# NoemieJaquier/GaBOtorch

Measured on AMD Instinct MI355X. Metric: SPD affine-invariant kernel-matrix build, pairs/sec (N=4096,d=10), higher is better.
Workload: dtype f64

## Files before the change

### gabotorch_amd/csrc/spd_pairwise_body.hpp

```cpp
#pragma once
#include "gabo_device.hpp"
#include "spd_eig.hpp"
#include "spd_prep.hpp"
#include "gabo_mirror.hpp"
#include "spd_generic.hpp"
#include "gabo_log_tab.hpp"
#include "gabo_exp_tab256.hpp"
#include "gabo_acosh2_table.hpp"
#include "../../include/gabo_hip.h"

#ifndef GABO_PAIR_WAVES
#define GABO_PAIR_WAVES 2
#endif

namespace gabo {

typedef const double __attribute__((address_space(1)))* spd_gcol_ptr;

struct SpdGcolBuffer {
    __amdgpu_buffer_rsrc_t rsrc;
    int voff;
    int stride_bytes;
    __device__ __forceinline__ double operator[](int k) const {
        return __builtin_bit_cast(double, __builtin_amdgcn_raw_buffer_load_b64(rsrc, voff, k * stride_bytes, 0));
    }
};
struct SpdGcolPointer {
    spd_gcol_ptr p;
    int64_t stride;
    __device__ __forceinline__ double operator[](int k) const { return p[(int64_t)k * stride]; }
};

template <int D, int ORIENT = kQlOrientPerLane, class GCOL>
__device__ __forceinline__ double ai_sumsq(const double* __restrict__ W, const GCOL& Gj, const double* __restrict__ ltab, const double eps2 = 0.0) {
    constexpr int T = tri_size(D);
    constexpr bool kDescending = ORIENT == kQlOrientLast;
    double m[T];
    static_for<D>([&](auto cc) {
        constexpr int col = kDescending ? D - 1 - decltype(cc)::value : decltype(cc)::value;
        double g[D - col], c[D - col];
        static_for<D - col>([&](auto kk) { g[decltype(kk)::value] = Gj[tri(col + decltype(kk)::value, col)]; });
        static_for<D - col>([&](auto rr) {
            constexpr int r = col + decltype(rr)::value;
            double acc = W[tri(r, col)] * g[0];
            static_for<r - col>([&](auto kk) {
                constexpr int k = col + 1 + decltype(kk)::value;
                acc = __builtin_fma(W[tri(r, k)], g[k - col], acc);
            });
            c[r - col] = acc;
        });
        static_for<D - col>([&](auto rr) {
            constexpr int r = col + decltype(rr)::value;
            static_for<r - col + 1>([&](auto qq) {
                constexpr int q = col + decltype(qq)::value;
                m[tri(r, q)] = (kDescending ? col == q : col == 0) ? c[r - col] * c[q - col] : __builtin_fma(c[r - col], c[q - col], m[tri(r, q)]);
            });
        });
    });
    double dg[D], e2[D];
    tridiagonalize<D, ORIENT>(m, dg, e2);
    tridiag_eigenvalues<D, ORIENT>(dg, e2, eps2);
    double s = 0.0;
    const LogTabRegs lr = LogTabRegs::load();
    static_for<D>([&](auto kk) { double lg = log_tab(dg[decltype(kk)::value], lr, ltab); s = __builtin_fma(lg, lg, s); });
    return s;
}

struct Spd2Col {
    double g00, g10, g11, lg;
};
__device__ __forceinline__ double ai_sumsq2(const double* __restrict__ W, const Spd2Col& g, double lw, const LogTabRegs& lr,
                                            const double* __restrict__ ltab, double tiny) {
    const double c00 = W[0] * g.g00, c11 = W[2] * g.g11;
    const double c10 = __builtin_fma(W[1], g.g00, W[2] * g.g10);
    const double m00 = c00 * c00, m10d = (c10 + c10) * c00, m11 = __builtin_fma(c10, c10, c11 * c11);
    const double tr = m00 + m11, df = m00 - m11;
    const double root = sqrt_nz(__builtin_fma(df, df, __builtin_fma(m10d, m10d, tiny)));
    const double l1 = log_tab(0.5 * (tr + root), lr, ltab);
    const double l2 = __builtin_fma(2.0, lw + g.lg, -l1);
    return __builtin_fma(l1, l1, l2 * l2);
}

__device__ __forceinline__ double finish(double dist, double beta, int mode) {
    if (mode == GABO_OUT_DISTANCE) return dist;
    if (mode == GABO_OUT_LAPLACE) return exp(-(dist * beta));
    return exp(-((dist * dist) * beta));
}

#ifndef GABO_PAIR_TWO_WAVE_MAX_DIM
#define GABO_PAIR_TWO_WAVE_MAX_DIM 14
#endif
#ifndef GABO_QL_EPS2_GAUSS
#define GABO_QL_EPS2_GAUSS 1e-14
#endif
constexpr bool spd_pair_gauss_only_instantiated(int d) { return d > 2 && d != 12; }
#ifndef GABO_PAIR_ORIENT
constexpr int spd_pair_gauss_only_orientation(int d) { return d == 14 ? kQlOrientCol0 : kQlOrientLast; }
#else
constexpr int spd_pair_gauss_only_orientation(int d) { return GABO_PAIR_ORIENT; }
#endif
template <int D, bool GAUSS_ONLY, bool BUFFER_ONLY>
__global__ __launch_bounds__(256, (D > GABO_PAIR_TWO_WAVE_MAX_DIM ? 1 : GABO_PAIR_WAVES)) void spd_ai_pairwise_kernel(const double* __restrict__ Winv, const double* __restrict__ G,
                                                              double* __restrict__ out, double* __restrict__ dist_out_arg,
                                                              int64_t n1, int64_t n2,
                                                              int64_t w_batch_stride, int64_t g_batch_stride, int rows,
                                                              int col_blocks, int row_chunks, int64_t sym_tiles, double beta, int flags) {
    constexpr int T = tri_size(D);
    static_assert(GAUSS_ONLY == BUFFER_ONLY && (spd_pair_gauss_only_instantiated(D) || !GAUSS_ONLY), "instantiations that launch_spd_ai selects");
    const int mode = GAUSS_ONLY ? GABO_OUT_GAUSSIAN : (flags & GABO_OUT_MASK);
    double* const dist_out = GAUSS_ONLY ? nullptr : dist_out_arg;
    constexpr bool kTabExp = D <= 4;
    __shared__ double tab[kTabExp ? 64 : 1];
    __shared__ __attribute__((aligned(16))) double ltab[512];
    for (int k = threadIdx.x; k < 512; k += blockDim.x) ltab[k] = kLogTab[k];
    double ec[6], ec3 = 0.0;
    if constexpr (kTabExp) {
        if (threadIdx.x < 64) tab[threadIdx.x] = kExp2Tab[threadIdx.x];
    }
    __syncthreads();
    if constexpr (kTabExp) {
        static_for<6>([&](auto k) { ec[decltype(k)::value] = kExpTabC[decltype(k)::value]; });
        ec3 = ec[3];
        asm volatile("" : "+v"(ec3));
    }
    int64_t cg, rc, b;
    if (flags & GABO_SYMMETRIC) {
        const int64_t per_batch = sym_tiles;
        b = blockIdx.x / per_batch;
        int64_t t = blockIdx.x - b * per_batch;
        cg = 0;
        for (;;) {
            int64_t cnt = ((cg + 1) * (int64_t)blockDim.x + rows - 1) / rows;
            if (cnt > row_chunks) cnt = row_chunks;
            if (t < cnt) break;
            t -= cnt;
            ++cg;
        }
        rc = t;
    } else {
        const int64_t bid = blockIdx.x;
        cg = bid % col_blocks;
        rc = (bid / col_blocks) % row_chunks;
        b = bid / ((int64_t)col_blocks * row_chunks);
    }
    const int64_t j0 = cg * blockDim.x;
    const int64_t j = j0 + threadIdx.x;
    const int64_t jc = j < n2 ? j : n2 - 1;
    const int64_t i0 = rc * rows;
    const int64_t i1 = (i0 + rows < n1) ? i0 + rows : n1;
    if ((flags & GABO_SYMMETRIC) && j0 + (int64_t)(threadIdx.x | 63) < i0) return;
    const double* Gj = G + b * g_batch_stride + jc;
    double* ob = out + b * n1 * n2;
    const int64_t jw = j0 + (threadIdx.x & ~63);
    const bool use_buffer = BUFFER_ONLY || (D > 2 && (int64_t)T * n2 * 8 < (1ll << 31));
    SpdGcolBuffer gbuf;
    {
        const double* gw = G + b * g_batch_stride + (jw < n2 ? jw : n2 - 1);
        uint64_t a = (uint64_t)gw;
        a = ((uint64_t)(uint32_t)__builtin_amdgcn_readfirstlane((int)(a >> 32)) << 32) | (uint32_t)__builtin_amdgcn_readfirstlane((int)a);
        gbuf.rsrc = __builtin_amdgcn_make_buffer_rsrc((void*)a, 0, 0x7fffffff, 0x00020000);
        gbuf.voff = (int)((jc - (jw < n2 ? jw : n2 - 1)) * 8);
        gbuf.stride_bytes = (int)(n2 * 8);
    }
    Spd2Col col2;
    double lw_lane = 0.0, tiny = 1e-290;
    LogTabRegs lr2;
    if constexpr (D == 2) {
        lr2 = LogTabRegs::load();
        asm volatile("" : "+s"(tiny));
        col2.g00 = Gj[0];
        col2.g10 = Gj[n2];
        col2.g11 = Gj[2 * n2];
        col2.lg = log_tab(col2.g00 * col2.g11, lr2, ltab);
        int64_t ir = i0 + (threadIdx.x & 63);
        ir = ir < n1 ? ir : n1 - 1;
        const double* Wr = Winv + b * w_batch_stride + ir * T;
        lw_lane = log_tab(Wr[0] * Wr[2], lr2, ltab);
    }
    double eps2 = (mode == GABO_OUT_GAUSSIAN && !dist_out) ? GABO_QL_EPS2_GAUSS : 0.0;
    asm volatile("" : "+s"(eps2));
    if constexpr (GAUSS_ONLY && BUFFER_ONLY) {
        const int nrows = __builtin_amdgcn_readfirstlane((int)(i1 - i0));
        const int64_t jrel = j - i0;
        const int rmax = j >= n2 ? -1 : ((flags & GABO_SYMMETRIC) ? (jrel < 0 ? -1 : (jrel > rows - 1 ? rows - 1 : (int)jrel)) : rows - 1);
        const double* W = Winv + b * w_batch_stride + i0 * T;
        char* orow = reinterpret_cast<char*>(ob + i0 * n2 + j);
        for (int r = 0; r < nrows; ++r, W += T) {
            SpdGcolBuffer gb = gbuf;
            asm volatile("" : "+v"(gb.voff));
            asm volatile("" : "+s"(gb.stride_bytes));
            const double s = ai_sumsq<D, spd_pair_gauss_only_orientation(D)>(W, gb, ltab, eps2);
            double val;
            if constexpr (kTabExp) {
                val = exp_neg_tab(-((s + 1e-15) * beta), ec, ec3, tab);
                val = s != s ? s : val;
            } else {
                val = exp(-((s + 1e-15) * beta));
            }
            if (r <= rmax) *reinterpret_cast<double*>(orow) = val;
            orow += (unsigned)gb.stride_bytes;
        }
        return;
    }
    for (int64_t i = i0; i < i1; ++i) {
        const double* W = Winv + b * w_batch_stride + i * T;
        double s;
        if constexpr (D == 2) {
            const int lane = (int)(i - i0);
            const double lw = __hiloint2double(__builtin_amdgcn_readlane(__double2hiint(lw_lane), lane),
                                               __builtin_amdgcn_readlane(__double2loint(lw_lane), lane));
            s = ai_sumsq2(W, col2, lw, lr2, ltab, tiny);
        } else {
            if (use_buffer) {
                SpdGcolBuffer gb = gbuf;
                asm volatile("" : "+v"(gb.voff));
                asm volatile("" : "+s"(gb.stride_bytes));
                s = ai_sumsq<D>(W, gb, ltab, eps2);
            } else {
                SpdGcolPointer gp{(spd_gcol_ptr)Gj, n2};
                asm volatile("" : "+v"(gp.p));
                s = ai_sumsq<D>(W, gp, ltab, eps2);
            }
        }
        double dist, val;
        if (mode == GABO_OUT_GAUSSIAN && !dist_out) {
            dist = 0.0;
            if constexpr (kTabExp) {
                val = exp_neg_tab(-((s + 1e-15) * beta), ec, ec3, tab);
                val = s != s ? s : val;
            } else {
                val = exp(-((s + 1e-15) * beta));
            }
        } else {
            dist = __builtin_sqrt(s + 1e-15);
            val = finish(dist, beta, mode);
        }
        if (j < n2 && (!(flags & GABO_SYMMETRIC) || i <= j)) {
            ob[i * n2 + j] = val;
            if (dist_out) dist_out[b * n1 * n2 + i * n2 + j] = dist;
        }
    }
}

#ifndef GABO_GAUSS2_MAX_ROWS
#define GABO_GAUSS2_MAX_ROWS 64
#endif
constexpr double kGauss2L = 0.0027076061740622863;
__constant__ double kGauss2C[6] = {kGauss2L, kGauss2L * kGauss2L / 2.0, kGauss2L * kGauss2L * kGauss2L / 6.0,
                                   kGauss2L * kGauss2L * kGauss2L * kGauss2L / 24.0, 6755399441055744.0, 4096.0};

template <bool NT, bool SYM>
__global__ __launch_bounds__(256) void spd_ai_gauss2_kernel(const double* __restrict__ Winv, const double* __restrict__ G,
                                                            double* __restrict__ out, int64_t n1, int64_t n2, int64_t w_batch_stride,
                                                            int64_t g_batch_stride, int rows, int col_blocks, int row_chunks,
                                                            int64_t sym_tiles, double beta, int flags) {
    __shared__ __attribute__((aligned(16))) double ltab[512];
    __shared__ double etab[256];
    __shared__ __attribute__((aligned(16))) double atab[kAcosh2Slots * kAcosh2Stride];
    __shared__ __attribute__((aligned(16))) double wrow[GABO_GAUSS2_MAX_ROWS * 4];
    const int tid = threadIdx.x;
    for (int k = tid; k < 512; k += blockDim.x) ltab[k] = kLogTab[k];
    for (int k = tid; k < 256; k += blockDim.x) etab[k] = kExp2Tab256[k];
    {
        const double sc = beta * (-512.0 / 0.69314718055994530942), eps = beta * (-256.0 / 0.69314718055994530942) * 1e-15;
        constexpr int kUsedLo = (kAcosh2Binades - 1) * 16 * kAcosh2Stride, kUsedHi = 240 * kAcosh2Stride;
        for (int k = tid; k < kAcosh2Slots * kAcosh2Stride - (kUsedHi - kUsedLo); k += blockDim.x) {
            const int kk = k < kUsedLo ? k : k + (kUsedHi - kUsedLo);
            const double v = kAcosh2Tab[kk] * sc;
            atab[kk] = (kk % kAcosh2Stride == 0) ? v + eps : v;
        }
    }
    int64_t cg, rc, b;
    if constexpr (SYM) {
        const int64_t per_batch = sym_tiles;
        b = blockIdx.x / per_batch;
        int64_t t = blockIdx.x - b * per_batch;
        cg = 0;
        for (;;) {
            int64_t cnt = ((cg + 1) * (int64_t)blockDim.x + rows - 1) / rows;
            if (cnt > row_chunks) cnt = row_chunks;
            if (t < cnt) break;
            t -= cnt;
            ++cg;
        }
        rc = t;
    } else {
        const int64_t bid = blockIdx.x;
        cg = bid % col_blocks;
        rc = (bid / col_blocks) % row_chunks;
        b = bid / ((int64_t)col_blocks * row_chunks);
    }
    const int64_t j0 = cg * blockDim.x;
    const int64_t j = j0 + tid;
    const int64_t jc = j < n2 ? j : n2 - 1;
    const int64_t i0 = rc * rows;
    const int64_t i1 = (i0 + rows < n1) ? i0 + rows : n1;
    const double* Gj = G + b * g_batch_stride + jc;
    const double g00 = Gj[0], g10 = Gj[n2], g11 = Gj[2 * n2];
    const LogTabRegs lr = LogTabRegs::load();
    const double sscale = __builtin_sqrt(beta * (512.0 / 0.69314718055994530942));
    double w0l = 1.0, w1l = 0.0, w2l = 1.0;
    if (tid < rows) {
        int64_t ir = i0 + tid;
        ir = ir < n1 ? ir : n1 - 1;
        const double* Wr = Winv + b * w_batch_stride + ir * 3;
        w0l = Wr[0], w1l = Wr[1], w2l = Wr[2];
    }
    __syncthreads();
    if (tid < rows) {
        const double dw = w0l * w2l;
        const double sw = rsqrt_nz(dw + dw);
        wrow[4 * tid + 0] = w0l * sw;
        wrow[4 * tid + 1] = w1l * sw;
        wrow[4 * tid + 2] = w2l * sw;
        wrow[4 * tid + 3] = sscale * log_tab(dw, lr, ltab);
    }
    __syncthreads();
    if (SYM && j0 + (int64_t)(tid | 63) < i0) return;
    double ec[6];
    static_for<6>([&](auto k) { ec[decltype(k)::value] = kGauss2C[decltype(k)::value]; });
    double c4v = ec[3];
    asm volatile("" : "+v"(c4v));
    const double dg = g00 * g11;
    const double bcol = sscale * log_tab(dg, lr, ltab);
    const double sg = rsqrt_nz(dg);
    const double q00 = g00 * sg, q10 = g10 * sg, q11 = g11 * sg;
    double* orow = out + b * n1 * n2 + i0 * n2 + j;
    const int nrows = __builtin_amdgcn_readfirstlane((int)(i1 - i0));
    const int64_t jrel = j - i0;
    const int rmax = j >= n2 ? -1 : (SYM ? (jrel < 0 ? -1 : (jrel > GABO_GAUSS2_MAX_ROWS - 1 ? GABO_GAUSS2_MAX_ROWS - 1 : (int)jrel)) : GABO_GAUSS2_MAX_ROWS - 1);
    typedef double g2_v2d __attribute__((ext_vector_type(2)));
    if (!SYM && j >= n2) return;
    for (int r = 0; r < nrows; ++r, orow += n2) {
        const g2_v2d wa = *reinterpret_cast<const g2_v2d*>(wrow + 4 * r);
        const g2_v2d wb = *reinterpret_cast<const g2_v2d*>(wrow + 4 * r + 2);
        const double w0 = wa[0], w1 = wa[1], w2 = wb[0], arow = wb[1];
        const double hh = __builtin_fma(w0, q00, -(w2 * q11));
        const double cc = __builtin_fma(w1, q00, w2 * q10);
        const double tau = __builtin_fma(cc, cc, __builtin_fma(hh, hh, 1.0));
        const unsigned hi = (unsigned)__double2hiint(tau);
        static_assert(kAcosh2MBits == 4 && kAcosh2Slots == 256, "row index = 8 bits");
        const unsigned off = __umul24((hi >> 16) & 0xffu, (unsigned)(kAcosh2Stride * sizeof(double)));
        const double t = tau - __hiloint2double((int)(hi & ~((1u << (20 - kAcosh2MBits)) - 1u)), 0);
        const g2_v2d* row = reinterpret_cast<const g2_v2d*>(reinterpret_cast<const char*>(atab) + off);
        static_assert(kAcosh2Deg == 7, "four coefficient pairs");
        const g2_v2d c67 = row[3], c45 = row[2], c23 = row[1], c01 = row[0];
        double ya = __builtin_fma(c67[1], t, c67[0]);
        ya = __builtin_fma(ya, t, c45[1]);
        ya = __builtin_fma(ya, t, c45[0]);
        ya = __builtin_fma(ya, t, c23[1]);
        ya = __builtin_fma(ya, t, c23[0]);
        ya = __builtin_fma(ya, t, c01[1]);
        ya = __builtin_fma(ya, t, c01[0]);
        if (__builtin_expect(__any(!(tau < ec[5])), 0)) {
            if (!(tau < ec[5])) {
                const double dl = log(tau + __builtin_sqrt(__builtin_fma(tau, tau, -1.0)));
                ya = -(sscale * sscale) * __builtin_fma(dl, dl, 0.5e-15);
            }
        }
        const double sp = arow + bcol;
        const double y = __builtin_fma(-sp, sp, ya);
        const double km = y + ec[4];
        const double kk = km - ec[4];
        const double rr = y - kk;
        double p = __builtin_fma(rr, c4v, ec[2]);
        p = __builtin_fma(p, rr, ec[1]);
        p = __builtin_fma(p, rr, ec[0]);
        p = p * rr;
        const int ki = __double2loint(km);
        const double e = etab[ki & 255];
        const double val = __builtin_ldexp(__builtin_fma(e, p, e), ki >> 8);
        if (!SYM || r <= rmax) {
            if constexpr (NT) __builtin_nontemporal_store(val, orow);
            else *orow = val;
        }
    }
}

template <int D>
static int launch_spd_ai(const double* x1, const double* x2, double* out, double* dist_out, int64_t batch, int64_t n1, int64_t n2,
                         int64_t s1, int64_t s2, double beta, int flags, double* ws, int* status, hipStream_t st, bool prepared = false) {
    constexpr int T = tri_size(D);
    const int64_t b1 = (s1 == 0) ? 1 : batch;
    const int64_t b2 = (s2 == 0) ? 1 : batch;
    double* W = ws;
    double* G = ws + b1 * n1 * T;
    if (!prepared) launch_spd_prep<D>(x1, x2, W, G, b1, b2, n1, n2, s1, s2, status, st, 1);
#ifndef GABO_PAIR_THREADS
#define GABO_PAIR_THREADS (D >= 7 ? 64 : 256)
#endif
    int threads = n2 >= 256 ? GABO_PAIR_THREADS : (n2 > 128 ? 192 : (n2 > 64 ? 128 : 64));
    int64_t col_blocks = (n2 + threads - 1) / threads;
#ifndef GABO_PAIR_ROWS_D2
#define GABO_PAIR_ROWS_D2 16
#endif
#ifndef GABO_PAIR_ROWS
#define GABO_PAIR_ROWS (D >= 9 ? 8 : 16)
#endif
#ifndef GABO_PAIR_ROWS_GAUSS2
#define GABO_PAIR_ROWS_GAUSS2 64
#endif
    const bool gauss2 = D == 2 && (flags & GABO_OUT_MASK) == GABO_OUT_GAUSSIAN && !dist_out && beta >= 0.0;
    int rows = D == 2 ? (gauss2 ? GABO_PAIR_ROWS_GAUSS2 : GABO_PAIR_ROWS_D2) : GABO_PAIR_ROWS;
    while (rows > 1 && col_blocks * ((n1 + rows - 1) / rows) * batch < (rows > 16 ? 1024 : 4096)) rows >>= 1;
    int64_t row_chunks = (n1 + rows - 1) / rows;
    int64_t sym_tiles = 0;
    if (flags & GABO_SYMMETRIC) {
        for (int64_t cg = 0; cg < col_blocks; ++cg) {
            int64_t cnt = ((cg + 1) * threads + rows - 1) / rows;
            sym_tiles += cnt < row_chunks ? cnt : row_chunks;
        }
    }
    int64_t nblocks = ((flags & GABO_SYMMETRIC) ? sym_tiles : col_blocks * row_chunks) * batch;
    if (nblocks > 0x7fffffffLL) return GABO_ERR_ARG;
    bool special2 = false;
    if constexpr (D == 2) special2 = gauss2 && rows <= GABO_GAUSS2_MAX_ROWS;
    if (special2) {
        const bool streaming = batch * n1 * n2 * 8 > (32ll << 20) && !(flags & GABO_SYMMETRIC);
#define GABO_GAUSS2_LAUNCH(...)                                                                                                     \
        hipLaunchKernelGGL((spd_ai_gauss2_kernel<__VA_ARGS__>), dim3((unsigned)nblocks), dim3(threads), 0, st, W, G, out, n1, n2,           \
                           (s1 == 0) ? (int64_t)0 : n1 * T, (s2 == 0) ? (int64_t)0 : n2 * T, rows, (int)col_blocks, (int)row_chunks,       \
                           sym_tiles, beta, flags)
        if (flags & GABO_SYMMETRIC) GABO_GAUSS2_LAUNCH(false, true);
        else if (streaming) GABO_GAUSS2_LAUNCH(true, false);
        else GABO_GAUSS2_LAUNCH(false, false);
#undef GABO_GAUSS2_LAUNCH
    } else {
#define GABO_PAIR_LAUNCH(...)                                                                                                             \
        hipLaunchKernelGGL((spd_ai_pairwise_kernel<D, __VA_ARGS__>), dim3((unsigned)nblocks), dim3(threads), 0, st, W, G, out, dist_out, n1, n2, \
                           (s1 == 0) ? (int64_t)0 : n1 * T, (s2 == 0) ? (int64_t)0 : n2 * T, rows, (int)col_blocks, (int)row_chunks,       \
                           sym_tiles, beta, flags)
        bool gauss_only = false;
        if constexpr (spd_pair_gauss_only_instantiated(D)) {
            gauss_only = (flags & GABO_OUT_MASK) == GABO_OUT_GAUSSIAN && !dist_out && (int64_t)T * n2 * 8 < (1ll << 31);
            if (gauss_only) GABO_PAIR_LAUNCH(true, true);
        }
        if (!gauss_only) GABO_PAIR_LAUNCH(false, false);
#undef GABO_PAIR_LAUNCH
    }
    if (flags & GABO_SYMMETRIC) {
        int tiles = (int)((n1 + 31) / 32);
        hipLaunchKernelGGL((mirror_upper_kernel<0>), dim3((unsigned)((int64_t)tiles * (tiles + 1) / 2), (unsigned)batch), dim3(256), 0, st,
                           out, n1, tiles);
        if (dist_out)
            hipLaunchKernelGGL((mirror_upper_kernel<0>), dim3((unsigned)((int64_t)tiles * (tiles + 1) / 2), (unsigned)batch), dim3(256), 0,
                               st, dist_out, n1, tiles);
    }
    return hipGetLastError() == hipSuccess ? GABO_OK : GABO_ERR_LAUNCH;
}

}

namespace gabo {
int launch_spd_ai_prepared(int d, double* out, int64_t batch, int64_t n1, int64_t n2, bool shared1, bool shared2, double beta, int flags,
                           double* ws, hipStream_t st);
int launch_spd_ai_wide2(int d, const double* x1, const double* x2, double* out, double* dist_out, int64_t batch, int64_t n1, int64_t n2,
                        int64_t s1, int64_t s2, double beta, int flags, double* ws, int* status, hipStream_t st);
int launch_spd_ai_wide3(int d, const double* x1, const double* x2, double* out, double* dist_out, int64_t batch, int64_t n1, int64_t n2,
                        int64_t s1, int64_t s2, double beta, int flags, double* ws, int* status, hipStream_t st);
int launch_spd_ai_wide(int d, const double* x1, const double* x2, double* out, double* dist_out, int64_t batch, int64_t n1, int64_t n2,
                       int64_t s1, int64_t s2, double beta, int flags, double* ws, int* status, hipStream_t st);
}
```

Baseline: 7.661 billion.

## Use 256-entry table exp and 3D grid in gaussian-only SPD pair kernel

For d=10 in the gaussian-only path, the libm exp is replaced by a 256-entry LDS table exp with a short polynomial, using scalar-register constants and beta folded into log2 units. Block indexing switches to a 3D grid so the div/mod decode is skipped. The log table fill uses vectorised loads issued before the LDS stores, and the row loop uses a countdown with a precomputed store threshold. The changes add LDS usage and rely on the accuracy of a low-order polynomial, and gauss_only is now limited to beta >= 0.

```diff
diff --git a/gabotorch_amd/csrc/spd_pairwise_body.hpp b/gabotorch_amd/csrc/spd_pairwise_body.hpp
--- a/gabotorch_amd/csrc/spd_pairwise_body.hpp
+++ b/gabotorch_amd/csrc/spd_pairwise_body.hpp
@@ -81,12 +81,49 @@
     return __builtin_fma(l1, l1, l2 * l2);
 }
 
+template <uint64_t BITS>
+__device__ __forceinline__ double scalar_const() {
+    int lo, hi;
+    asm volatile("s_mov_b32 %0, %1" : "=s"(lo) : "n"((int)(uint32_t)BITS));
+    asm volatile("s_mov_b32 %0, %1" : "=s"(hi) : "n"((int)(uint32_t)(BITS >> 32)));
+    return __hiloint2double(hi, lo);
+}
+__device__ __forceinline__ double fma_scalar_addend(double a, double b, double c_uniform) {
+    double r;
+    asm("v_fma_f64 %0, %1, %2, %3" : "=v"(r) : "v"(a), "v"(b), "s"(c_uniform));
+    return r;
+}
+constexpr double kPairExpL = 0.0027076061740622863;
+__device__ __forceinline__ double exp_tab256_units(double y, const double* __restrict__ etab) {
+    y = max_raw(y, scalar_const<__builtin_bit_cast(uint64_t, -294912.0)>());
+    const double magic = scalar_const<__builtin_bit_cast(uint64_t, 6755399441055744.0)>();
+    const double km = y + magic;
+    const double k = km - magic;
+    const double r = y - k;
+    constexpr double c4 = __builtin_bit_cast(double, __builtin_bit_cast(uint64_t, kPairExpL * kPairExpL * kPairExpL * kPairExpL / 24.0) & 0xffffffff00000000ull);
+    double p = fma_scalar_addend(r, c4, scalar_const<__builtin_bit_cast(uint64_t, kPairExpL * kPairExpL * kPairExpL / 6.0)>());
+    p = fma_scalar_addend(p, r, scalar_const<__builtin_bit_cast(uint64_t, kPairExpL * kPairExpL / 2.0)>());
+    p = fma_scalar_addend(p, r, scalar_const<__builtin_bit_cast(uint64_t, kPairExpL)>());
+    p = p * r;
+    const int ki = __double2loint(km);
+    const double e = etab[ki & 255];
+    return __builtin_ldexp(__builtin_fma(e, p, e), ki >> 8);
+}
+
 __device__ __forceinline__ double finish(double dist, double beta, int mode) {
     if (mode == GABO_OUT_DISTANCE) return dist;
     if (mode == GABO_OUT_LAPLACE) return exp(-(dist * beta));
     return exp(-((dist * dist) * beta));
 }
 
+#ifndef GABO_PAIR_GRID3D
+#define GABO_PAIR_GRID3D 1
+#endif
+#ifndef GABO_PAIR_EXP256
+constexpr bool spd_pair_gauss_only_table_exp(int d) { return d == 10; }
+#else
+constexpr bool spd_pair_gauss_only_table_exp(int d) { return GABO_PAIR_EXP256 && d >= 5; }
+#endif
 #ifndef GABO_PAIR_TWO_WAVE_MAX_DIM
 #define GABO_PAIR_TWO_WAVE_MAX_DIM 14
 #endif
@@ -110,21 +147,16 @@
     const int mode = GAUSS_ONLY ? GABO_OUT_GAUSSIAN : (flags & GABO_OUT_MASK);
     double* const dist_out = GAUSS_ONLY ? nullptr : dist_out_arg;
     constexpr bool kTabExp = D <= 4;
+    constexpr bool kExp256 = GAUSS_ONLY && !kTabExp && spd_pair_gauss_only_table_exp(D);
     __shared__ double tab[kTabExp ? 64 : 1];
+    __shared__ __attribute__((aligned(16))) double etab[kExp256 ? 256 : 2];
     __shared__ __attribute__((aligned(16))) double ltab[512];
-    for (int k = threadIdx.x; k < 512; k += blockDim.x) ltab[k] = kLogTab[k];
-    double ec[6], ec3 = 0.0;
-    if constexpr (kTabExp) {
-        if (threadIdx.x < 64) tab[threadIdx.x] = kExp2Tab[threadIdx.x];
-    }
-    __syncthreads();
-    if constexpr (kTabExp) {
-        static_for<6>([&](auto k) { ec[decltype(k)::value] = kExpTabC[decltype(k)::value]; });
-        ec3 = ec[3];
-        asm volatile("" : "+v"(ec3));
-    }
     int64_t cg, rc, b;
-    if (flags & GABO_SYMMETRIC) {
+    if (GABO_PAIR_GRID3D && col_blocks == 0) {
+        cg = blockIdx.x;
+        rc = blockIdx.y;
+        b = blockIdx.z;
+    } else if (flags & GABO_SYMMETRIC) {
         const int64_t per_batch = sym_tiles;
         b = blockIdx.x / per_batch;
         int64_t t = blockIdx.x - b * per_batch;
@@ -148,9 +180,40 @@
     const int64_t jc = j < n2 ? j : n2 - 1;
     const int64_t i0 = rc * rows;
     const int64_t i1 = (i0 + rows < n1) ? i0 + rows : n1;
-    if ((flags & GABO_SYMMETRIC) && j0 + (int64_t)(threadIdx.x | 63) < i0) return;
     const double* Gj = G + b * g_batch_stride + jc;
     double* ob = out + b * n1 * n2;
+    typedef double spd_v2d __attribute__((ext_vector_type(2)));
+    {
+        constexpr int kLsteps = 4, kEsteps = kExp256 ? 2 : 0;
+        spd_v2d lv[kLsteps], ev[kEsteps ? kEsteps : 1];
+        static_for<kLsteps>([&](auto uu) {
+            const int k = (int)threadIdx.x + decltype(uu)::value * (int)blockDim.x;
+            lv[decltype(uu)::value] = reinterpret_cast<const spd_v2d*>(kLogTab)[k < 255 ? k : 255];
+        });
+        static_for<kEsteps>([&](auto uu) {
+            const int k = (int)threadIdx.x + decltype(uu)::value * (int)blockDim.x;
+            ev[decltype(uu)::value] = reinterpret_cast<const spd_v2d*>(kExp2Tab256)[k < 127 ? k : 127];
+        });
+        static_for<kLsteps>([&](auto uu) {
+            const int k = (int)threadIdx.x + decltype(uu)::value * (int)blockDim.x;
+            if (k < 256) reinterpret_cast<spd_v2d*>(ltab)[k] = lv[decltype(uu)::value];
+        });
+        static_for<kEsteps>([&](auto uu) {
+            const int k = (int)threadIdx.x + decltype(uu)::value * (int)blockDim.x;
+            if (k < 128) reinterpret_cast<spd_v2d*>(etab)[k] = ev[decltype(uu)::value];
+        });
+    }
+    double ec[6], ec3 = 0.0;
+    if constexpr (kTabExp) {
+        if (threadIdx.x < 64) tab[threadIdx.x] = kExp2Tab[threadIdx.x];
+    }
+    __syncthreads();
+    if constexpr (kTabExp) {
+        static_for<6>([&](auto k) { ec[decltype(k)::value] = kExpTabC[decltype(k)::value]; });
+        ec3 = ec[3];
+        asm volatile("" : "+v"(ec3));
+    }
+    if ((flags & GABO_SYMMETRIC) && j0 + (int64_t)(threadIdx.x | 63) < i0) return;
     const int64_t jw = j0 + (threadIdx.x & ~63);
     const bool use_buffer = BUFFER_ONLY || (D > 2 && (int64_t)T * n2 * 8 < (1ll << 31));
     SpdGcolBuffer gbuf;
@@ -185,7 +248,13 @@
         const int rmax = j >= n2 ? -1 : ((flags & GABO_SYMMETRIC) ? (jrel < 0 ? -1 : (jrel > rows - 1 ? rows - 1 : (int)jrel)) : rows - 1);
         const double* W = Winv + b * w_batch_stride + i0 * T;
         char* orow = reinterpret_cast<char*>(ob + i0 * n2 + j);
-        for (int r = 0; r < nrows; ++r, W += T) {
+        double beta_units = beta * (-256.0 / 0.69314718055994530942);
+        if constexpr (kExp256)
+            beta_units = __hiloint2double(__builtin_amdgcn_readfirstlane(__double2hiint(beta_units)), __builtin_amdgcn_readfirstlane(__double2loint(beta_units)));
+        uint64_t ostep = (unsigned)gbuf.stride_bytes;
+        if constexpr (kExp256) asm volatile("" : "+v"(ostep));
+        const int left_min = nrows - rmax;
+        for (int left = nrows; left > 0; --left, W += T) {
             SpdGcolBuffer gb = gbuf;
             asm volatile("" : "+v"(gb.voff));
             asm volatile("" : "+s"(gb.stride_bytes));
@@ -194,11 +263,14 @@
             if constexpr (kTabExp) {
                 val = exp_neg_tab(-((s + 1e-15) * beta), ec, ec3, tab);
                 val = s != s ? s : val;
+            } else if constexpr (kExp256) {
+                val = exp_tab256_units((s + scalar_const<__builtin_bit_cast(uint64_t, 1e-15)>()) * beta_units, etab);
+                val = __hiloint2double(s != s ? __double2hiint(s) : __double2hiint(val), __double2loint(val));
             } else {
                 val = exp(-((s + 1e-15) * beta));
             }
-            if (r <= rmax) *reinterpret_cast<double*>(orow) = val;
-            orow += (unsigned)gb.stride_bytes;
+            if (left >= left_min) *reinterpret_cast<double*>(orow) = val;
+            orow += ostep;
         }
         return;
     }
@@ -413,6 +485,8 @@
     }
     int64_t nblocks = ((flags & GABO_SYMMETRIC) ? sym_tiles : col_blocks * row_chunks) * batch;
     if (nblocks > 0x7fffffffLL) return GABO_ERR_ARG;
+    const bool grid3 = GABO_PAIR_GRID3D && !(flags & GABO_SYMMETRIC) && row_chunks <= 65535 && batch <= 65535;
+    const dim3 pair_grid = grid3 ? dim3((unsigned)col_blocks, (unsigned)row_chunks, (unsigned)batch) : dim3((unsigned)nblocks);
     bool special2 = false;
     if constexpr (D == 2) special2 = gauss2 && rows <= GABO_GAUSS2_MAX_ROWS;
     if (special2) {
@@ -427,12 +501,12 @@
 #undef GABO_GAUSS2_LAUNCH
     } else {
 #define GABO_PAIR_LAUNCH(...)                                                                                                             \
-        hipLaunchKernelGGL((spd_ai_pairwise_kernel<D, __VA_ARGS__>), dim3((unsigned)nblocks), dim3(threads), 0, st, W, G, out, dist_out, n1, n2, \
-                           (s1 == 0) ? (int64_t)0 : n1 * T, (s2 == 0) ? (int64_t)0 : n2 * T, rows, (int)col_blocks, (int)row_chunks,       \
+        hipLaunchKernelGGL((spd_ai_pairwise_kernel<D, __VA_ARGS__>), pair_grid, dim3(threads), 0, st, W, G, out, dist_out, n1, n2,            \
+                           (s1 == 0) ? (int64_t)0 : n1 * T, (s2 == 0) ? (int64_t)0 : n2 * T, rows, grid3 ? 0 : (int)col_blocks, (int)row_chunks, \
                            sym_tiles, beta, flags)
         bool gauss_only = false;
         if constexpr (spd_pair_gauss_only_instantiated(D)) {
-            gauss_only = (flags & GABO_OUT_MASK) == GABO_OUT_GAUSSIAN && !dist_out && (int64_t)T * n2 * 8 < (1ll << 31);
+            gauss_only = (flags & GABO_OUT_MASK) == GABO_OUT_GAUSSIAN && !dist_out && (int64_t)T * n2 * 8 < (1ll << 31) && beta >= 0.0;
             if (gauss_only) GABO_PAIR_LAUNCH(true, true);
         }
         if (!gauss_only) GABO_PAIR_LAUNCH(false, false);
```

Result: no change. 7.731 billion (median of 6 runs) (+0.9%).
